# ericyao2013/path_planning_2d

Hardware: AMD Instinct MI355X
Metric: grid cells/sec for belief-update+Bellman loop, 1024x1024; plan step p50 ms (higher is better)
Workload: dtype fp32; 1 GPU; 1024x1024 cells per GPU: 1 belief update + 1 MDP Bellman sweep per step (BASELINE.json configs[2] grid); rows_per_gpu=1024, parallelism=single GPU, cells_per_lane=4, model=dictionary-coded (274 entries, uint16 code per cell)

## Files before the change

### path_planning_2d_amd/csrc/pp2_resident.hip

```cpp
#include <algorithm>
#include <cstring>
#include <type_traits>

#include "pp2_coded_dev.h"

namespace pp2 {

#ifdef PP2_RES_TRACE
__device__ unsigned long long g_rtrace[16][64][4][4];
#define PP2_RT(ph)                                                                    \
  if (tile < 16 && t < 64 && lane == 0 && (wave == 0 || wave == 5 || wave == 9 || wave == 12)) \
  g_rtrace[tile][t][wave == 0 ? 0 : wave == 5 ? 1 : wave == 9 ? 2 : 3][ph] =          \
      __builtin_amdgcn_s_memrealtime()
__device__ unsigned long long g_rtrace_pro[1024][8];
#define PP2_RP(ph) \
  if (tile < 1024 && threadIdx.x == 0) g_rtrace_pro[tile][ph] = __builtin_amdgcn_s_memrealtime()
#else
#define PP2_RT(ph) (void)0
#define PP2_RP(ph) (void)0
#endif

namespace {

typedef __amdgpu_buffer_rsrc_t Rsrc;
// ... 239 lines not shown
    if (sl < 0) continue;
#pragma unroll
    for (int k = 0; k < 4; ++k)
      p[k] = __builtin_fmaf(*reinterpret_cast<const float*>(qr + 4 * sl + cb[wr][k + 1 + wc]),
                            win.v[wr][k + 1 + wc], p[k]);
  }
#pragma unroll
  for (int k = 0; k < 4; ++k)
    p[k] = p[k] * *reinterpret_cast<const float*>(lt + __builtin_amdgcn_ubfe(lx4, 8 * k, 8));
}
__device__ __forceinline__ void belief_any_regs(int u, const ClassRegs& cr, uint32_t lx4, int z,
                                                const Win6& w, float (&p)[4]) {
  switch (u) {
#define PP2_BQ(UU)                               \
  case UU:                                       \
    belief_fact_regs<UU>(cr, lx4, z, w, p);      \
    break;
    PP2_BQ(0) PP2_BQ(1) PP2_BQ(2) PP2_BQ(3) PP2_BQ(4) PP2_BQ(5) PP2_BQ(6) PP2_BQ(7)
    default: belief_fact_regs<8>(cr, lx4, z, w, p);
#undef PP2_BQ
  }
}
__device__ __forceinline__ void load_class_regs(const uint8_t* sP, int prows, int ps, int ty,
                                                int x0, ClassRegs& cr) {
  const int lane = threadIdx.x & 63;
#pragma unroll
  for (int U = 0; U < 9; ++U)
#pragma unroll
    for (int oy = 0; oy < 3; ++oy) {
      const int sl = kCls.s[U][oy];
      if (sl < 0) continue;
      const uint8_t* r = sP + (U * prows + ty + oy) * ps + 4 + x0;
      const uint32_t m = *reinterpret_cast<const uint32_t*>(r);
      uint32_t e = 0u;
      if (lane == 0 || lane == 63) e = *reinterpret_cast<const uint32_t*>(r + (lane == 0 ? -4 : 4));
      const uint32_t l = (uint32_t)__builtin_amdgcn_update_dpp((int)e, (int)m, 0x138, 0xf, 0xf, false);
      const uint32_t h = (uint32_t)__builtin_amdgcn_update_dpp((int)e, (int)m, 0x130, 0xf, 0xf, false);
      cr.m[sl] = m;
      const uint32_t lh = (l >> 24) | ((h & 0xffu) << 8);
      cr.lh[sl / 2] = (sl & 1) ? cr.lh[sl / 2] | (lh << 16) : lh;
    }
}

template <bool TR>
__device__ __forceinline__ void belief_any(int u, const uint8_t* sP, int prows, int ps, int ty,
                                           int x0, uint32_t lx4, int z, const Win6& w,
                                           float (&p)[4]) {
  int off = (u * prows + ty) * ps;
  asm("" : "+v"(off));
  const uint8_t* pu = sP + off;
  switch (u) {
#define PP2_BQ(UU)                                                     \
  case UU:                                                             \
    belief_fact<UU, TR>(pu, ps, x0, lx4, z, w, p); \
    break;
    PP2_BQ(0) PP2_BQ(1) PP2_BQ(2) PP2_BQ(3) PP2_BQ(4) PP2_BQ(5) PP2_BQ(6) PP2_BQ(7)
    default: belief_fact<8, TR>(pu, ps, x0, lx4, z, w, p);
#undef PP2_BQ
  }
}
__device__ __forceinline__ const uint8_t* class_rows_of(int u, const uint8_t* sP, int prows, int ps,
                                                        int ty) {
  int off = (u * prows + ty) * ps;
  asm("" : "+v"(off));
  return sP + off;
}
template <bool TR>
__device__ __forceinline__ void belief_any_pre(int u, int x0, uint32_t lx4, int z, const Win6& w,
                                               const ClassRows& c, float (&p)[4]) {
  switch (u) {
#define PP2_BQ(UU)                                                  \
  case UU:                                                          \
    belief_fact<UU, TR, true>(nullptr, 0, x0, lx4, z, w, p, &c);    \
    break;
    PP2_BQ(0) PP2_BQ(1) PP2_BQ(2) PP2_BQ(3) PP2_BQ(4) PP2_BQ(5) PP2_BQ(6) PP2_BQ(7)
    default: belief_fact<8, TR, true>(nullptr, 0, x0, lx4, z, w, p, &c);
#undef PP2_BQ
  }
}

#ifndef PP2_RES_MASKED
#define PP2_RES_MASKED 1
#endif
template <int U>
__device__ __forceinline__ void belief_masked(float wm, float ws, const float (&tc)[4],
                                              const float (&lz)[4], const float (&mk)[4],
                                              const float (&bo)[4], const Win6& win,
                                              float (&p)[4]) {
#pragma unroll
  for (int k = 0; k < 4; ++k) p[k] = 0.0f;
#pragma unroll
  for (int s = 0; s < 9; ++s) {
    const int wr = s / 3, wc = s % 3 - 1, i = 8 - s;
    if (kSupSlot.s[U][i] < 0) continue;
#pragma unroll
    for (int k = 0; k < 4; ++k) {
      const float wt = i == 4 ? tc[k] : i == U ? wm : ws;
      p[k] = __builtin_fmaf(wt, win.v[wr][k + 1 + wc], p[k]);
    }
  }
#pragma unroll
  for (int k = 0; k < 4; ++k) {
    const float own = __builtin_fmaf(tc[k], bo[k], 0.0f);
    p[k] = (mk[k] == 0.0f ? own : p[k]) * lz[k];
  }
}
[[maybe_unused]] __device__ __forceinline__ void belief_any_masked(
    int u, float wm, float ws, const float (&tc)[4], const float (&lz)[4], const float (&mk)[4],
    const float (&bo)[4], const Win6& w, float (&p)[4]) {
  switch (u) {
#define PP2_BQ(UU)                                        \
  case UU:                                                \
    belief_masked<UU>(wm, ws, tc, lz, mk, bo, w, p);      \
    break;
    PP2_BQ(0) PP2_BQ(1) PP2_BQ(2) PP2_BQ(3) PP2_BQ(4) PP2_BQ(5) PP2_BQ(6) PP2_BQ(7)
    default: belief_masked<8>(wm, ws, tc, lz, mk, bo, w, p);
#undef PP2_BQ
  }
}
struct CentreSlots {
  unsigned long long v;
  constexpr CentreSlots() : v(0) {
    for (int u = 0; u < 9; ++u) v |= (unsigned long long)(4 * sup_slot(u, 4)) << (4 * u);
  }
};
constexpr CentreSlots kCentreSlot{};

__device__ __forceinline__ void row_lds(const float* row, int x0, float (&v)[6]) {
  const float* p = row + x0;
  const f4a m = *reinterpret_cast<const f4a*>(p);
  const int lane = threadIdx.x & 63;
  float e = 0.0f;
  if (lane == 0 || lane == 63) e = p[lane == 0 ? -1 : 4];
  v[0] = __int_as_float(__builtin_amdgcn_update_dpp(__float_as_int(e), __float_as_int(m[3]),
                                                    0x138, 0xf, 0xf, false));
  v[1] = m[0]; v[2] = m[1]; v[3] = m[2]; v[4] = m[3];
  v[5] = __int_as_float(__builtin_amdgcn_update_dpp(__float_as_int(e), __float_as_int(m[0]),
                                                    0x130, 0xf, 0xf, false));
}
__device__ __forceinline__ void row_zero(float (&v)[6]) {
#pragma unroll
  for (int i = 0; i < 6; ++i) v[i] = 0.0f;
}
#ifndef PP2_RES_WINDOW1
#define PP2_RES_WINDOW1 2
#endif
#ifndef PP2_RES_SWEEP_WINDOW1
#define PP2_RES_SWEEP_WINDOW1 PP2_RES_WINDOW1
#endif
#if PP2_RES_WINDOW1 != 0 || PP2_RES_SWEEP_WINDOW1 != 0
template <int NP>
struct WinRows {
  f4a q[NP][3];
  float e[NP][3];
};
template <int MODE, int NP>
__device__ __forceinline__ void issue_window_rows(const float* const (&p)[NP], int xs, bool in0,
                                                  bool in2, WinRows<NP>& w) {
  const int lane = threadIdx.x & 63;
#pragma unroll
  for (int k = 0; k < NP; ++k) w.q[k][1] = *reinterpret_cast<const f4a*>(p[k]);
  if (in0) {
#pragma unroll
    for (int k = 0; k < NP; ++k) w.q[k][0] = *reinterpret_cast<const f4a*>(p[k] - xs);
  }
  if (in2) {
#pragma unroll
    for (int k = 0; k < NP; ++k) w.q[k][2] = *reinterpret_cast<const f4a*>(p[k] + xs);
  }
  const int o0 = in0 ? -xs : 0, o2 = in2 ? xs : 0;
  auto edges = [&](int eo) {
#pragma unroll
    for (int k = 0; k < NP; ++k) w.e[k][2] = p[k][o2 + eo];
#pragma unroll
    for (int k = 0; k < NP; ++k) w.e[k][1] = p[k][eo];
#pragma unroll
    for (int k = NP - 1; k >= 0; --k) w.e[k][0] = p[k][o0 + eo];
  };
  if constexpr (MODE == 1) {
#pragma unroll
    for (int k = 0; k < NP; ++k)
#pragma unroll
      for (int r = 0; r < 3; ++r) w.e[k][r] = 0.0f;
    if (lane == 0 || lane == 63) edges(lane == 0 ? -1 : 4);
  } else {
    edges(lane < 32 ? -1 - 4 * lane : 4 + 4 * (63 - lane));
  }
}
__device__ __forceinline__ void window_row(const f4a& m, float e, float (&v)[6]) {
  v[0] = __int_as_float(__builtin_amdgcn_update_dpp(__float_as_int(e), __float_as_int(m[3]),
                                                    0x138, 0xf, 0xf, false));
  v[1] = m[0]; v[2] = m[1]; v[3] = m[2]; v[4] = m[3];
  v[5] = __int_as_float(__builtin_amdgcn_update_dpp(__float_as_int(e), __float_as_int(m[0]),
                                                    0x130, 0xf, 0xf, false));
}
#endif

__device__ __forceinline__ int xch_gran(int ntiles, int wpr, int slot, int tl, int side, int w,
                                        int k, int ln) {
  return (((((slot * ntiles + tl) * 2 + side) * wpr + w) * kResidentGranules + k) * 64 + ln) * 16;
}
#ifndef PP2_RES_XCD_PLAIN
#define PP2_RES_XCD_PLAIN 1
#endif
#ifndef PP2_RES_EARLY
#define PP2_RES_EARLY 2
#endif
#ifndef PP2_RES_REDW0
#define PP2_RES_REDW0 1
#endif
#ifndef PP2_RES_XCD_AUX
#define PP2_RES_XCD_AUX 0
#endif
__device__ __forceinline__ int tile_xcd(int t, int n) {
  const int q = n / 8, r = n % 8;
  return t < r * (q + 1) ? t / (q + 1) : r + (q > 0 ? (t - r * (q + 1)) / q : 0);
}
__device__ __forceinline__ void st_quad_x(Rsrc r, int off, const float (&v)[4], unsigned bit,
                                          bool plain) {
  const unsigned m = bit << 31;
  const u4v t = {__float_as_uint(v[0]) | m, __float_as_uint(v[1]) | m, __float_as_uint(v[2]) | m,
                 __float_as_uint(v[3]) | m};
  if (plain) __builtin_amdgcn_raw_buffer_store_b128(t, r, off, 0, PP2_RES_XCD_AUX);
  else __builtin_amdgcn_raw_buffer_store_b128(t, r, off, 0, kSc1);
}
__device__ __forceinline__ bool tagged(const u4v& g, unsigned m) {
  return (((g[0] ^ m) | (g[1] ^ m) | (g[2] ^ m) | (g[3] ^ m)) >> 31) == 0u;
}
__device__ __forceinline__ float untag(unsigned w) { return __uint_as_float(w & 0x7fffffffu); }
template <int NG>
__device__ __forceinline__ void take_granules(Rsrc r, int o, bool edge, int eo, unsigned bit,
                                              u4v (&g)[NG], unsigned (&e)[NG], unsigned* err,
                                              unsigned* err_host) {
  const unsigned m = bit << 31;
  const unsigned long long t0 = wall_clock64();
#pragma unroll
  for (int k = 0; k < NG; ++k) e[k] = m;
  for (int spin = 0;; ++spin) {
#pragma unroll
    for (int k = 0; k < NG; ++k) g[k] = __builtin_amdgcn_raw_buffer_load_b128(r, o + 1024 * k, 0, kSc1);
    if (edge) {
#pragma unroll
      for (int k = 0; k < NG; ++k) e[k] = __builtin_amdgcn_raw_buffer_load_b32(r, eo + 1024 * k, 0, kSc1);
    }
    bool ok = true;
#pragma unroll
    for (int k = 0; k < NG; ++k) ok = ok && tagged(g[k], m) && ((e[k] ^ m) >> 31) == 0u;
    if (__all(ok)) break;
    if ((spin & 7) == 7) {
      if (ld_flag(err) != 0u || wall_clock64() - t0 > kSpinTicks) {
        if ((threadIdx.x & 63) == 0) raise_err(err, err_host);
        return;
      }
    }
    __builtin_amdgcn_s_sleep(1);
    asm volatile("" ::: "memory");
  }
}
typedef unsigned u2v __attribute__((ext_vector_type(2)));
__device__ __forceinline__ int side_gran(int sbase, int ntiles, int slot, int tl, int side, int r) {
  return sbase + (((slot * ntiles + tl) * 2 + side) * kResidentMaxRt + r) * 8;
}
__device__ __forceinline__ void st_pair(Rsrc r, int off, float b, float j, unsigned bit) {
  const unsigned m = bit << 31;
  const u2v t = {__float_as_uint(b) | m, __float_as_uint(j) | m};
  __builtin_amdgcn_raw_buffer_store_b64(t, r, off, 0, kSc1);
}
__device__ __forceinline__ void take_rows_sides(Rsrc r, bool rows, int o, bool edge, int eo,
                                                bool sd, const int (&so)[3], int soff, unsigned bit,
                                                u4v (&g)[2], unsigned (&e)[2], u2v (&s)[3],
                                                unsigned* err, unsigned* err_host) {
  const unsigned m = bit << 31;
  const unsigned long long t0 = wall_clock64();
  e[0] = e[1] = m;
#pragma unroll
  for (int k = 0; k < 3; ++k) s[k] = u2v{m, m};
#ifdef PP2_RES_NOXCH
  g[0] = g[1] = u4v{m, m, m, m};
  return;
#endif
  for (int spin = 0;; ++spin) {
    if (rows) {
      g[0] = __builtin_amdgcn_raw_buffer_load_b128(r, o, 0, kSc1);
      g[1] = __builtin_amdgcn_raw_buffer_load_b128(r, o + 1024, 0, kSc1);
      if (edge) {
        e[0] = __builtin_amdgcn_raw_buffer_load_b32(r, eo, 0, kSc1);
        e[1] = __builtin_amdgcn_raw_buffer_load_b32(r, eo + 1024, 0, kSc1);
      }
    }
    if (sd) {
#pragma unroll
      for (int k = 0; k < 3; ++k)
        if (so[k] >= 0) s[k] = __builtin_amdgcn_raw_buffer_load_b64(r, so[k], soff, kSc1);
    }
    bool ok = true;
    if (rows)
      ok = tagged(g[0], m) && tagged(g[1], m) && (((e[0] ^ m) | (e[1] ^ m)) >> 31) == 0u;
#pragma unroll
    for (int k = 0; k < 3; ++k) ok = ok && (((s[k][0] ^ m) | (s[k][1] ^ m)) >> 31) == 0u;
#ifdef PP2_RES_NOWAIT
    ok = true;
#endif
    if (__all(ok)) break;
    if ((spin & 7) == 7) {
      if (ld_flag(err) != 0u || wall_clock64() - t0 > kSpinTicks) {
        if ((threadIdx.x & 63) == 0) raise_err(err, err_host);
        return;
      }
    }
    __builtin_amdgcn_s_sleep(1);
    asm volatile("" ::: "memory");
  }
}
__device__ __forceinline__ void row_quad(const float (&m)[4], float e, float (&v)[6]) {
  v[0] = __int_as_float(__builtin_amdgcn_update_dpp(__float_as_int(e), __float_as_int(m[3]),
                                                    0x138, 0xf, 0xf, false));
  v[1] = m[0]; v[2] = m[1]; v[3] = m[2]; v[4] = m[3];
  v[5] = __int_as_float(__builtin_amdgcn_update_dpp(__float_as_int(e), __float_as_int(m[0]),
                                                    0x130, 0xf, 0xf, false));
}

template <int CAP>
struct alignas(4) Trajectory {
  static_assert(CAP % 4 == 0, "the loop reads the trajectory as 32-bit words");
  uint8_t uz[CAP];
};

__device__ __forceinline__ ResidentMasked masked_arg() { return ResidentMasked{}; }
[[maybe_unused]] __device__ __forceinline__ ResidentMasked masked_arg(const ResidentMasked& m) {
  return m;
}
template <int CAP, int TC, bool LAG, bool TR, class... MW>
__global__ __launch_bounds__(TC == 3 ? 768 : 1024, TC == 3 ? 3 : 4) void k_loop_resident(
    const ResidentHead a, const Trajectory<CAP> tr, const MW... mwa) {
  static_assert(!TR || TC == 1, "transposed tiles are whole kernel rows");
  constexpr bool MSK = sizeof...(MW) != 0;
  static_assert(!MSK || (TC == 1 && !LAG && !TR), "the masked form is a whole-row instance");
  const ResidentMasked mw = masked_arg(mwa...);
  (void)mw;
  constexpr int kSweepG = TC == 3 ? 4 : TC > 1 ? 2 : 0;
  constexpr bool kSweepPipe = TC == 1 && !LAG && !TR;
  extern __shared__ __attribute__((aligned(16))) float lds[];
  constexpr int tc = TC == 3 ? 2 : TC;
  const int wp = a.g.wp, rows = a.g.rows, tw = wp / tc;
  const int tpr = tw >> 2, wpr = tw >> 8;
  const int xs = tw + 4;
  const int bufn = 4 + a.rt * xs;
  const int prows = a.rt + 2, ps = tw + 8;
  float* sTC = lds + lds_span(kResTab);
  uint8_t* sP = reinterpret_cast<uint8_t*>(sTC + lds_span(rows_floats(a.E, true)));
  float* sB0 = reinterpret_cast<float*>(sP) + lds_span(MSK ? kResGCn : 9 * prows * ps / 4);
  const float* sGC = reinterpret_cast<const float*>(sP);
  (void)sGC;
  float* sS = sB0 + 4 * bufn;
  float* sRed = sS + 16;

  const int tile = xcd_remap(blockIdx.x, gridDim.x);
  if (tile == a.stall_tile) return;
  const int trow = tile / tc, cx = tile - trow * tc, gx = cx * tw;
  PP2_RP(0);
  const unsigned prior_err = ld_flag(a.sync + kResidentSyncErr);
  const int lane = threadIdx.x & 63, wave = threadIdx.x >> 6;
  const int ty = __builtin_amdgcn_readfirstlane(threadIdx.x / tpr);
  const int wraw = __builtin_amdgcn_readfirstlane((threadIdx.x % tpr) >> 6);
  const int wj = tc > 1 ? __builtin_amdgcn_readfirstlane((wraw + ty) % wpr) : wraw;
  const int x0 = wj * 256 + lane * 4;
  const int y = trow * a.rt + ty;
  const bool valid = y < rows;
  const bool own = TR ? x0 >= a.own0 && x0 < a.own1 : y >= a.own0 && y < a.own1;
  auto hoff = [&](int yy, int xx) -> long long {
    return TR ? (long long)xx * a.ows + yy : (long long)yy * wp + xx;
  };
  const bool nb_up = valid && ty == 0 && trow > 0;
  const bool nb_dn = valid && ty == a.rt - 1 && y + 1 < rows;
  const bool sd_l = valid && wj == 0 && cx > 0;
  const bool sd_r = valid && wj == wpr - 1 && cx + 1 < tc;
  const bool sd_lane = (sd_l && lane == 0) || (sd_r && lane == 63);
  const int sbase = 2 * a.ntiles * 2 * (wp >> 8) * kResidentGranules * 64 * 16;
  unsigned* const err = a.sync + kResidentSyncErr;
  const Rsrc rx = make_rsrc(a.xch);
  auto sbuf = [&](int k, int slot) { return sB0 + (2 * k + slot) * bufn + 4; };
  const int myx = tile_xcd(tile, (int)gridDim.x);
  const bool plain_up = PP2_RES_XCD_PLAIN && nb_up && tile_xcd(tile - tc, (int)gridDim.x) == myx;
  const bool plain_dn = PP2_RES_XCD_PLAIN && nb_dn && tile_xcd(tile + tc, (int)gridDim.x) == myx;
  auto publish = [&](int slot, const float (&b)[4], const float (&j)[4], unsigned bit) {
#pragma unroll
    for (int side = 0; side < 2; ++side) {
      if (side == 0 ? !nb_up : !nb_dn) continue;
      const int o = xch_gran(a.ntiles, wpr, slot, tile, side, wj, 0, lane);
      const bool plain = side == 0 ? plain_up : plain_dn;
      st_quad_x(rx, o, b, bit, plain);
      st_quad_x(rx, o + 1024, j, bit, plain);
    }
    if (sd_lane) {
      const int o = side_gran(sbase, a.ntiles, slot, tile, sd_l ? 0 : 1, ty);
      if (sd_l) st_pair(rx, o, b[0], j[0], bit);
      else st_pair(rx, o, b[3], j[3], bit);
    }
  };
  int so[3] = {-1, -1, -1};
  if (tc > 1 && sd_lane) {
    const int dir = sd_l ? -1 : 1, nside = sd_l ? 1 : 0;
#pragma unroll
    for (int k = 0; k < 3; ++k) {
      const int rr = ty + k - 1, yy = y + k - 1;
      if (yy < 0 || yy >= rows) continue;
      const int tl2 = rr < 0 ? tile - tc + dir : rr >= a.rt ? tile + tc + dir : tile + dir;
      so[k] = side_gran(sbase, a.ntiles, 0, tl2, nside, rr < 0 ? a.rt - 1 : rr >= a.rt ? 0 : rr);
    }
  }
  const int sslot = a.ntiles * 2 * kResidentMaxRt * 8;
  auto take = [&](int slot, bool rows_in, int tl, int side, bool sd, unsigned bit, float (&vb)[6],
                  float (&vj)[6], float (&sb)[3], float (&sj)[3]) {
    const bool el = lane == 0 && wj > 0, er = lane == 63 && wj + 1 < wpr;
    const int o = xch_gran(a.ntiles, wpr, slot, tl, side, wj, 0, lane);
    const int eo = el ? xch_gran(a.ntiles, wpr, slot, tl, side, wj - 1, 0, 63) + 12
                      : xch_gran(a.ntiles, wpr, slot, tl, side, wj + 1, 0, 0);
    u4v g[2];
    unsigned e[2];
    u2v s[3];
    take_rows_sides(rx, rows_in, o, el || er, eo, sd && sd_lane, so, slot * sslot, bit, g, e, s,
                    err, a.err_host);
    if (rows_in) {
      const float mb[4] = {untag(g[0][0]), untag(g[0][1]), untag(g[0][2]), untag(g[0][3])};
      const float mj[4] = {untag(g[1][0]), untag(g[1][1]), untag(g[1][2]), untag(g[1][3])};
      row_quad(mb, (el || er) ? untag(e[0]) : 0.0f, vb);
      row_quad(mj, (el || er) ? untag(e[1]) : 0.0f, vj);
    }
    if (sd) {
#pragma unroll
      for (int k = 0; k < 3; ++k) {
        sb[k] = untag(s[k][0]);
        sj[k] = untag(s[k][1]);
      }
    }
  };

  const bool start0 = a.kstep0 % a.depth == 0;
  const bool red0 = start0 && a.in_partials && wave == 0;
  const bool red0_regs = red0 && a.in_n <= kPrologueParts;
  f4a pq[kPrologueParts / 256];
  if (red0_regs) {
    const f4a* q = reinterpret_cast<const f4a*>(a.in_partials);
    const int nq = a.in_n >> 2;
#pragma unroll
    for (int j = 0; j < kPrologueParts / 256; ++j) {
      const int i = lane + 64 * j;
      pq[j] = q[i < nq ? i : 0];
    }
  }
  f4a b_t = {0.0f, 0.0f, 0.0f, 0.0f}, j_t = {0.0f, 0.0f, 0.0f, 0.0f};
  if (valid) {
    if (TR) {
#pragma unroll
      for (int k = 0; k < 4; ++k) {
        b_t[k] = a.b_in[hoff(y, x0 + k)];
        j_t[k] = a.j_in[hoff(y, x0 + k)];
      }
    } else {
      const long long off = (long long)y * wp + gx + x0;
      b_t = *reinterpret_cast<const f4a*>(a.b_in + off);
      j_t = *reinterpret_cast<const f4a*>(a.j_in + off);
    }
  }
  stage_rows(a.rfact, kResTab, lds);
  stage_rows(a.rows, rows_floats(a.E, true), sTC);
  if constexpr (MSK) stage_rows(a.rfact + kResGC, kResGCn, reinterpret_cast<float*>(sP));
  for (int i = threadIdx.x; i < 4 * (a.rt + 1); i += blockDim.x) {
    const int buf = i / (a.rt + 1), r = i % (a.rt + 1);
    *reinterpret_cast<f4a*>(sB0 + buf * bufn + r * xs) = f4a{0.0f, 0.0f, 0.0f, 0.0f};
  }
  uint32_t cc[4] = {0u, 0u, 0u, 0u}, iwr[4][3], lx4 = 0u;
  if (valid) {
    if (TR) {
#pragma unroll
      for (int k = 0; k < 4; ++k) cc[k] = a.code[hoff(y, x0 + k)];
    } else {
      const uint2 m = *reinterpret_cast<const uint2*>(a.code + (long long)y * wp + gx + x0);
      cc[0] = m.x & 0xffffu; cc[1] = m.x >> 16; cc[2] = m.y & 0xffffu; cc[3] = m.y >> 16;
    }
    const uint8_t* lx = reinterpret_cast<const uint8_t*>(a.rfact + kResLX);
#pragma unroll
    for (int k = 0; k < 4; ++k) lx4 |= (uint32_t)lx[cc[k]] << (8 * k);
  }
  float mk[4] = {1.0f, 1.0f, 1.0f, 1.0f};
  if constexpr (MSK) {
    if (valid) {
      const uint8_t* fx = reinterpret_cast<const uint8_t*>(a.rfact + kResFX);
#pragma unroll
      for (int k = 0; k < 4; ++k) mk[k] = fx[cc[k]] ? 0.0f : 1.0f;
    }
  }
  __syncthreads();
  PP2_RP(1);
#pragma unroll
  for (int k = 0; k < 4; ++k) {
    const uint4 w = *reinterpret_cast<const uint4*>(sTC + kFactIW + 4 * cc[k]);
    iwr[k][0] = w.x; iwr[k][1] = w.y; iwr[k][2] = w.z;
  }
  for (int i = threadIdx.x; !MSK && i < prows * tpr; i += blockDim.x) {
    const int r = i / tpr, xq = (i % tpr) * 4, yy = trow * a.rt + r - 1;
    uint32_t pl[9] = {0u, 0u, 0u, 0u, 0u, 0u, 0u, 0u, 0u};
    if (yy >= 0 && yy < rows) {
      uint32_t c4[4];
      if (TR) {
#pragma unroll
        for (int k = 0; k < 4; ++k) c4[k] = a.code[hoff(yy, xq + k)];
      } else {
        const uint2 m = *reinterpret_cast<const uint2*>(a.code + (long long)yy * wp + gx + xq);
        c4[0] = m.x & 0xffffu; c4[1] = m.x >> 16; c4[2] = m.y & 0xffffu; c4[3] = m.y >> 16;
      }
#pragma unroll
      for (int k = 0; k < 4; ++k) {
        const uint4 w = *reinterpret_cast<const uint4*>(sTC + kFactIW + 4 * c4[k]);
#pragma unroll
        for (int q = 0; q < 9; ++q) {
          const uint32_t wq = q < 4 ? w.x : q < 8 ? w.y : w.z;
          pl[q] |= __builtin_amdgcn_ubfe(wq, 8 * (q % 4), 8) << (8 * k);
        }
      }
    }
#pragma unroll
    for (int q = 0; q < 9; ++q)
      *reinterpret_cast<uint32_t*>(sP + (q * prows + r) * ps + 4 + xq) = pl[q];
  }
  for (int i = threadIdx.x; !MSK && i < 9 * prows; i += blockDim.x) {
    const int q = i / prows, yy = trow * a.rt + i % prows - 1;
    uint32_t lp = 0u, rp = 0u;
    if (yy >= 0 && yy < rows) {
      auto cls = [&](int x) {
        const uint4 w = *reinterpret_cast<const uint4*>(
            sTC + kFactIW + 4 * a.code[hoff(yy, x)]);
        return __builtin_amdgcn_ubfe(q < 4 ? w.x : q < 8 ? w.y : w.z, 8 * (q % 4), 8);
      };
      if (gx > 0) lp = cls(gx - 1) << 24;
      if (gx + tw < wp) rp = cls(gx + tw);
    }
    *reinterpret_cast<uint32_t*>(sP + i * ps) = lp;
    *reinterpret_cast<uint32_t*>(sP + i * ps + 4 + tw) = rp;
  }
  PP2_RP(4);
  ClassRegs creg;
  if constexpr (TC == 3 && PP2_RES_HOIST) {
    __syncthreads();
    if (valid) load_class_regs(sP, prows, ps, ty, x0, creg);
  }
  if (prior_err != 0u) return;
  const bool bnd = nb_up || nb_dn || sd_l || sd_r;
  if (valid) {
    f4a b = b_t, j = j_t;
    if constexpr (MSK) {
      *reinterpret_cast<f4a*>(sbuf(0, 1) + ty * xs + x0) = b;
      *reinterpret_cast<f4a*>(sbuf(1, 1) + ty * xs + x0) = j;
#pragma unroll
      for (int k = 0; k < 4; ++k) {
        b[k] = b[k] * mk[k];
        j[k] = j[k] * mk[k];
      }
    }
    *reinterpret_cast<f4a*>(sbuf(0, 0) + ty * xs + x0) = b;
    *reinterpret_cast<f4a*>(sbuf(1, 0) + ty * xs + x0) = j;
    if (bnd) {
      const float bv[4] = {b[0], b[1], b[2], b[3]}, jv[4] = {j[0], j[1], j[2], j[3]};
      publish(1, bv, jv, (a.slot_use[1] + 1u) & 1u);
    }
  }
  unsigned use[2] = {a.slot_use[0], a.slot_use[1] + 1u};
  PP2_RP(5);
  if constexpr (kSweepPipe && PP2_RES_EARLY == 2) {
    if (threadIdx.x == 0) sS[1] = 0.0f;
  }
  if (red0) {
    float S;
    if (red0_regs) {
      const int nq = a.in_n >> 2;
      float sl = 0.0f;
#pragma unroll
      for (int j = 0; j < kPrologueParts / 256; ++j)
        if (lane + 64 * j < nq) sl += ((pq[j][0] + pq[j][1]) + pq[j][2]) + pq[j][3];
      S = wave_sum(sl);
    } else {
      S = wave_reduce_partials(a.in_partials, a.in_n);
    }
    if (threadIdx.x == 0) {
      sS[0] = S;
      if (tile == 0 && a.in_sum_out) *a.in_sum_out = S;
    }
  }
  __syncthreads();
  float inv = 1.0f;
  if (start0)
    inv = (1.0f / (a.in_partials ? sS[0] : a.in_sum ? *a.in_sum : 1.0f)) * a.bscale;

  const int pi = y * (wp >> 8) + cx * wpr + wj;
  const int redw = kSweepPipe && PP2_RES_REDW0 != 0 ? 0 : a.rt >= 3 && wpr >= 4 ? wpr + 1 : 0;
  unsigned arrivals = a.arrive_base;
  const unsigned nvw = kSweepPipe ? (unsigned)(std::min(a.rt, rows - trow * a.rt) * wpr) : 0u;
  unsigned early_n = 0u;
  (void)nvw;
  (void)early_n;
  int shift = 0;
  constexpr bool lag = LAG;
  int sh_prev = 0;
  unsigned arr_v = 0u;
  bool red_ok = false;
  auto lag_start = [&](int T) {
    return lag && T > 0 && T < a.n && T % a.depth == 0 && T - 1 - a.depth >= 0;
  };
  auto lag_target = [&](int T) { return a.arrive_base + (unsigned)(T / a.depth - 1) * a.ntiles; };
  float p[4] = {0.0f, 0.0f, 0.0f, 0.0f}, best[4] = {0.0f, 0.0f, 0.0f, 0.0f}, local = 0.0f;
  uint32_t arg[4] = {0u, 0u, 0u, 0u};
  if constexpr (MSK) {
    if (valid) {
      const f4a b = *reinterpret_cast<const f4a*>(sbuf(0, 1) + ty * xs + x0);
      const f4a j = *reinterpret_cast<const f4a*>(sbuf(1, 1) + ty * xs + x0);
#pragma unroll
      for (int k = 0; k < 4; ++k) {
        p[k] = b[k];
        best[k] = j[k];
      }
    }
  }
  PP2_RP(2);

  const uint32_t* const trw = reinterpret_cast<const uint32_t*>(tr.uz);
  uint32_t uzw = trw[0];
  int ph = a.kstep0 % a.depth;
  (void)trw;
  (void)uzw;
  (void)ph;
  for (int t = 0; t < a.n; ++t) {
#if PP2_RES_TRAJ_SGPR
    const uint32_t uzb = (uzw >> (8 * (t & 3))) & 0xffu;
    const int u = uzb & 15, z = uzb >> 4;
#else
    const int u = tr.uz[t] & 15, z = tr.uz[t] >> 4;
#endif
    const int ci = t & 1, co = ci ^ 1;
    const bool last = t == a.n - 1;
#if PP2_RES_PHASE_CTR
    const bool bs = t > 0 && ph == 0;
    ph = ph + 1 == a.depth ? 0 : ph + 1;
#else
    const bool bs = t > 0 && (a.kstep0 + t) % a.depth == 0;
#endif
    if (t > 0 && !bs) inv = 1.0f;
    if (lag) {
      if (wave == redw) {
        if (lag_start(t + 1)) {
          red_ok = a.red_lds && reached(arr_v, lag_target(t + 1));
          if (red_ok) {
            const float* src = a.ring + (size_t)((t - a.depth) % kResidentRing) * a.nparts;
            const int nq = a.nparts >> 2;
            for (int c = 0; c * 64 < nq; ++c) {
              const int i = c * 64 + lane < nq ? c * 64 + lane : nq - 1;
              __builtin_amdgcn_global_load_lds((glb_void*)(src + 4 * i), (lds_void*)(sRed + c * 256), 16,
                                               0, kSc1);
            }
          }
        }
        if (lag_start(t + 2)) arr_v = ld_flag(a.sync + kResidentSyncArrive);
      }
      if (bs) {
        const int sh = t - 1 - a.depth >= 0 ? pow2_shift_lagged(sS[0], sh_prev)
                       : start0 && (a.in_partials || a.in_sum) ? pow2_shift_lagged(a.bscale, 0)
                                                               : 0;
        sh_prev = sh;
        shift += sh;
        inv = pow2f(sh);
      }
    }
    PP2_RT(0);
    local = 0.0f;
#if PP2_RES_PHASE_CTR
    const bool arrive = ph == 0;
#else
    const bool arrive = (a.kstep0 + t + 1) % a.depth == 0;
#endif
    const bool mass = !kSweepPipe || arrive || last;
    const bool early = kSweepPipe && PP2_RES_EARLY != 0 && arrive && !bs && !last &&
                       !(t == 0 && start0);
    auto early_arrive = [&]() {
      float s = 0.0f;
#pragma unroll
      for (int k = 0; k < 4; ++k) s += p[k];
      const float v = wave_sum(s);
      if (lane == 0 && pi < a.nparts)
        st_flag(reinterpret_cast<unsigned*>(a.ring + (size_t)(t % kResidentRing) * a.nparts + pi),
                __float_as_uint(v));
      asm volatile("s_waitcnt vmcnt(0)" ::: "memory");
#if PP2_RES_EARLY == 1
      __syncthreads();
      if (threadIdx.x == 0)
        __hip_atomic_fetch_add(a.sync + kResidentSyncArrive, 1u, __ATOMIC_RELAXED,
                               __HIP_MEMORY_SCOPE_AGENT);
#else
      early_n += nvw;
      if (lane == 0) {
        const unsigned old = __hip_atomic_fetch_add(reinterpret_cast<unsigned*>(sS + 1), 1u,
                                                    __ATOMIC_RELAXED, __HIP_MEMORY_SCOPE_WORKGROUP);
        if (old + 1u == early_n)
          __hip_atomic_fetch_add(a.sync + kResidentSyncArrive, 1u, __ATOMIC_RELAXED,
                                 __HIP_MEMORY_SCOPE_AGENT);
      }
      asm volatile("" ::: "memory");
#endif
    };
    auto step_quad = [&]() {
      Win6 wb, wj;
      float sb[3] = {0.0f, 0.0f, 0.0f}, sj[3] = {0.0f, 0.0f, 0.0f};
      const bool sd = sd_l || sd_r;
      const unsigned bit = use[co] & 1u;
      ClassRows crow;
      if constexpr (kSweepPipe && !MSK)
        load_class_rows(class_rows_of(u, sP, prows, ps, ty), ps, x0, crow);
      float rtv[2][4][4], rcost[2][4];
      if constexpr (kSweepPipe && !MSK) {
        if (last) coded_sweep_iw_pipe_begin<4, true>(sTC, iwr, rtv, rcost, best, arg);
        else coded_sweep_iw_pipe_begin<4, false>(sTC, iwr, rtv, rcost, best, arg);
      }
      float tcv[4], lzv[4], mrec[2][4][2];
      if constexpr (MSK) {
        const char* qr = reinterpret_cast<const char*>(lds + kResQR) + u * (kFactK * 16) +
                         (int)((kCentreSlot.v >> (4 * u)) & 15u);
        const char* lt = reinterpret_cast<const char*>(lds + kResLT) + z * (kResLK * 4);
        const uint32_t sel0 = 0x0c0c0c00u | (uint32_t)(u & 7);
        const uint32_t sel1 = 0x0c0c0c00u | (u == 8 ? 4u : 0u);
#pragma unroll
        for (int k = 0; k < 4; ++k) {
          const uint32_t lo = __builtin_amdgcn_perm(iwr[k][1], iwr[k][0], sel0);
          tcv[k] = *reinterpret_cast<const float*>(qr + __builtin_amdgcn_perm(iwr[k][2], lo, sel1));
        }
#pragma unroll
        for (int k = 0; k < 4; ++k)
          lzv[k] = *reinterpret_cast<const float*>(lt + __builtin_amdgcn_ubfe(lx4, 8 * k, 8));
        if (last) masked_sweep_pipe_begin<4, true>(sGC, iwr, mrec);
        else masked_sweep_pipe_begin<4, false>(sGC, iwr, mrec);
      }
#if PP2_RES_WINDOW1 != 0
      if constexpr (kSweepPipe) {
        const bool in0 = ty > 0, in2 = ty + 1 < a.rt && y + 1 < rows;
        WinRows<2> wr;
        const float* const wp2[2] = {sbuf(0, ci) + ty * xs + x0, sbuf(1, ci) + ty * xs + x0};
        issue_window_rows<PP2_RES_WINDOW1>(wp2, xs, in0, in2, wr);
        __builtin_amdgcn_sched_barrier(0);
        if (in0) {
          window_row(wr.q[0][0], wr.e[0][0], wb.v[0]);
          window_row(wr.q[1][0], wr.e[1][0], wj.v[0]);
        } else if (nb_up) {
          take(co, true, tile - tc, 1, sd, bit, wb.v[0], wj.v[0], sb, sj);
        } else {
          row_zero(wb.v[0]);
          row_zero(wj.v[0]);
        }
        window_row(wr.q[0][1], wr.e[0][1], wb.v[1]);
        window_row(wr.q[1][1], wr.e[1][1], wj.v[1]);
        if (in2) {
          window_row(wr.q[0][2], wr.e[0][2], wb.v[2]);
          window_row(wr.q[1][2], wr.e[1][2], wj.v[2]);
        } else if (nb_dn) {
          take(co, true, tile + tc, 0, sd && !nb_up, bit, wb.v[2], wj.v[2], sb, sj);
        } else {
          row_zero(wb.v[2]);
          row_zero(wj.v[2]);
        }
      } else
#endif
      {
        if (ty > 0) {
          row_lds(sbuf(0, ci) + (ty - 1) * xs, x0, wb.v[0]);
          row_lds(sbuf(1, ci) + (ty - 1) * xs, x0, wj.v[0]);
        } else if (nb_up) {
          take(co, true, tile - tc, 1, sd, bit, wb.v[0], wj.v[0], sb, sj);
        } else {
          row_zero(wb.v[0]);
          row_zero(wj.v[0]);
        }
        row_lds(sbuf(0, ci) + ty * xs, x0, wb.v[1]);
        row_lds(sbuf(1, ci) + ty * xs, x0, wj.v[1]);
        if (ty + 1 < a.rt && y + 1 < rows) {
          row_lds(sbuf(0, ci) + (ty + 1) * xs, x0, wb.v[2]);
          row_lds(sbuf(1, ci) + (ty + 1) * xs, x0, wj.v[2]);
        } else if (nb_dn) {
          take(co, true, tile + tc, 0, sd && !nb_up, bit, wb.v[2], wj.v[2], sb, sj);
        } else {
          row_zero(wb.v[2]);
          row_zero(wj.v[2]);
        }
      }
      if (sd && !nb_up && !nb_dn) take(co, false, tile, 0, true, bit, wb.v[1], wj.v[1], sb, sj);
      if (sd_lane) {
#pragma unroll
        for (int k = 0; k < 3; ++k) {
          if (sd_l) {
            wb.v[k][0] = sb[k];
            wj.v[k][0] = sj[k];
          } else {
            wb.v[k][5] = sb[k];
            wj.v[k][5] = sj[k];
          }
        }
      }
      PP2_RT(1);
      if constexpr (TC == 3 && PP2_RES_HOIST) {
#pragma unroll
        for (int i = 0; i < kClsSlots; ++i) asm volatile("" : "+v"(creg.m[i]));
#pragma unroll
        for (int i = 0; i < (kClsSlots + 1) / 2; ++i) asm volatile("" : "+v"(creg.lh[i]));
        belief_any_regs(u, creg, lx4, z, wb, p);
      }
      else if constexpr (MSK) {
        const float bo[4] = {p[0], p[1], p[2], p[3]};
        belief_any_masked(u, mw.w_main, mw.w_side, tcv, lzv, mk, bo, wb, p);
        if constexpr (PP2_RES_EARLY != 0) {
          if (early) early_arrive();
        }
      }
      else if constexpr (kSweepPipe) {
        belief_any_pre<TR>(u, x0, lx4, z, wb, crow, p);
        if constexpr (PP2_RES_EARLY != 0) {
          if (early) early_arrive();
        }
      }
      else belief_any<TR>(u, sP, prows, ps, ty, x0, lx4, z, wb, p);
      float jn[9][4];
#pragma unroll
      for (int i = 0; i < 9; ++i)
#pragma unroll
        for (int k = 0; k < 4; ++k) jn[i][k] = TR ? wj.v[i % 3][k + i / 3] : wj.v[i / 3][k + i % 3];
      if constexpr (MSK) {
        float ov[4] = {best[0], best[1], best[2], best[3]};
        if (last)
          masked_sweep_pipe_rest<4, true>(sGC, iwr, jn, mw.gw_main, mw.gw_side, mrec, ov, best, arg);
        else
          masked_sweep_pipe_rest<4, false>(sGC, iwr, jn, mw.gw_main, mw.gw_side, mrec, ov, best, arg);
#pragma unroll
        for (int k = 0; k < 4; ++k) {
          const bool blocked = mk[k] == 0.0f;
          best[k] = blocked ? ov[k] : best[k];
          arg[k] = blocked ? 0u : arg[k];
        }
        *reinterpret_cast<f4a*>(sbuf(1, co) + ty * xs + x0) =
            f4a{best[0] * mk[0], best[1] * mk[1], best[2] * mk[2], best[3] * mk[3]};
        return;
      } else if constexpr (kSweepPipe) {
        if (last) coded_sweep_iw_pipe_rest<4, true>(sTC, iwr, jn, rtv, rcost, best, arg);
        else coded_sweep_iw_pipe_rest<4, false>(sTC, iwr, jn, rtv, rcost, best, arg);
      } else {
        if (last) coded_sweep_iw<4, true, kSweepG>(sTC, iwr, jn, best, arg);
        else coded_sweep_iw<4, false, kSweepG>(sTC, iwr, jn, best, arg);
      }
      *reinterpret_cast<f4a*>(sbuf(1, co) + ty * xs + x0) = f4a{best[0], best[1], best[2], best[3]};
    };
    auto finish_quad = [&]() {
#pragma unroll
      for (int k = 0; k < 4; ++k) p[k] = p[k] * inv;
      if (mass && !early) {
#pragma unroll
        for (int k = 0; k < 4; ++k) local += p[k];
      }
      if constexpr (MSK) {
        const float pm[4] = {p[0] * mk[0], p[1] * mk[1], p[2] * mk[2], p[3] * mk[3]};
        *reinterpret_cast<f4a*>(sbuf(0, co) + ty * xs + x0) = f4a{pm[0], pm[1], pm[2], pm[3]};
        if (bnd) {
          const float jm[4] = {best[0] * mk[0], best[1] * mk[1], best[2] * mk[2], best[3] * mk[3]};
          if (!last) publish(ci, pm, jm, (use[ci] + 1u) & 1u);
          __builtin_amdgcn_s_setprio(0);
        }
        return;
      }
      *reinterpret_cast<f4a*>(sbuf(0, co) + ty * xs + x0) = f4a{p[0], p[1], p[2], p[3]};
      if (bnd) {
        if (!last) publish(ci, p, best, (use[ci] + 1u) & 1u);
        __builtin_amdgcn_s_setprio(0);
      }
    };
    if (valid) {
      if (bnd) __builtin_amdgcn_s_setprio(2);
      step_quad();
      if (!bs || lag) finish_quad();
    }
#if PP2_RES_EARLY == 1
    else if (early) __syncthreads();
#endif
    if (bs && !lag) {
      if (wave == redw) {
        arrivals += a.ntiles;
        wave_wait(a.sync + kResidentSyncArrive, 1, arrivals, err, a.err_host);
        const float S = wave_reduce_partials_sc1(
            a.ring + (size_t)((t - 1) % kResidentRing) * a.nparts, a.nparts);
        if (lane == 0) sS[0] = S;
      }
      __syncthreads();
      if (a.shard) {
        const int sh = pow2_shift(sS[0]);
        shift += sh;
        inv = pow2f(sh);
      } else {
        inv = (1.0f / sS[0]) * a.bscale;
      }
      if (valid) finish_quad();
    }
    PP2_RT(2);
    if (last) break;
    ++use[ci];
    if (mass && !early) {
      const float v = wave_sum(local);
      if (lane == 0 && pi < a.nparts)
        st_flag(reinterpret_cast<unsigned*>(a.ring + (size_t)(t % kResidentRing) * a.nparts + pi),
                __float_as_uint(v));
    }
    if (arrive && !early) asm volatile("s_waitcnt vmcnt(0)" ::: "memory");
    if (wave == redw && lag_start(t + 1)) {
      float S;
      if (red_ok) {
        const int nq = a.nparts >> 2;
        float sl = 0.0f;
        for (int i = lane; i < nq; i += 64) {
          const f4a w = *reinterpret_cast<const f4a*>(sRed + 4 * i);
          sl += ((w[0] + w[1]) + w[2]) + w[3];
        }
        S = wave_sum(sl);
      } else {
        wave_wait(a.sync + kResidentSyncArrive, 1, lag_target(t + 1), err, a.err_host);
        S = wave_reduce_partials_sc1(a.ring + (size_t)((t - a.depth) % kResidentRing) * a.nparts,
                                     a.nparts);
      }
      if (lane == 0) sS[0] = S;
    }
#if PP2_RES_TRAJ_SGPR
    if (((t + 1) & 3) == 0 && t + 1 < CAP) uzw = trw[(t + 1) >> 2];
#endif
#ifndef PP2_RES_NOBAR
    __syncthreads();
#endif
    if (arrive && !early && threadIdx.x == 0)
      __hip_atomic_fetch_add(a.sync + kResidentSyncArrive, 1u, __ATOMIC_RELAXED,
                             __HIP_MEMORY_SCOPE_AGENT);
    PP2_RT(3);
  }

  if (own && TR) {
#pragma unroll
    for (int k = 0; k < 4; ++k) {
      const long long off = hoff(y, x0 + k);
      __builtin_nontemporal_store(p[k], a.b_out + off);
      __builtin_nontemporal_store(best[k], a.j_out + off);
      a.A[off] = (uint8_t)arg[k];
    }
  } else if (own) {
    const long long off = (long long)y * wp + gx + x0;
    store4<true>(a.b_out + off, p);
    store_ja<true>(a.j_out, a.A, off, best, arg);
  }
  const float v = wave_sum(own ? local : 0.0f);
  if (lane == 0 && pi < a.nparts) a.out_partials[pi] = v;
  if (a.scale_out && tile == 0 && threadIdx.x == 0) *a.scale_out = shift;
  PP2_RP(3);
}


__global__ __launch_bounds__(1024, 4) void k_sweep_resident(const SweepRun a) {
  extern __shared__ __attribute__((aligned(16))) float lds[];
  const int wp = a.g.wp, rows = a.g.rows, tpr = wp >> 2, wpr = wp >> 8;
  const int xs = wp + 4;
  const int bufn = 4 + a.rt * xs;
  float* sTC = lds;
  float* sJ0 = sTC + lds_span(rows_floats(a.E, true));
  float* sM = sJ0 + 3 * bufn;

  const int tile = xcd_remap(blockIdx.x, gridDim.x);
  if (tile == a.stall_tile) return;
  const unsigned prior_err = ld_flag(a.sync + kResidentSyncErr);
  const int lane = threadIdx.x & 63, wave = threadIdx.x >> 6;
  const int ty = __builtin_amdgcn_readfirstlane(threadIdx.x / tpr);
  const int wj = __builtin_amdgcn_readfirstlane((threadIdx.x % tpr) >> 6);
  const int x0 = (threadIdx.x % tpr) * 4;
// ... 106 lines not shown
      else if (nb_dn) take(co, tile + 1, 0, use[co] & 1u, w.v[2]);
      else row_zero(w.v[2]);
      float jn[9][4];
#pragma unroll
      for (int i = 0; i < 9; ++i)
#pragma unroll
        for (int k = 0; k < 4; ++k) jn[i][k] = w.v[i / 3][k + i % 3];
      if (check || fin) coded_sweep_iw_pipe<4, true>(sTC, iwr, jn, best, arg);
      else coded_sweep_iw_pipe<4, false>(sTC, iwr, jn, best, arg);
#endif
      *reinterpret_cast<f4a*>(sbuf(co) + ty * xs + x0) = f4a{best[0], best[1], best[2], best[3]};
      if (nb_up || nb_dn) {
        publish(ci, best, (use[ci] + 1u) & 1u);
        __builtin_amdgcn_s_setprio(0);
      }
    }
    ++use[ci];
    if (fin) break;
    if (!check) {
      __syncthreads();
      continue;
    }
    float m = 0.0f;
    if (valid) {
      float* sn = sbuf(2) + ty * xs + x0;
      const f4a old = *reinterpret_cast<const f4a*>(sn);
#pragma unroll
      for (int k = 0; k < 4; ++k) m = fmaxf(m, fabsf(old[k] - best[k]));
      *reinterpret_cast<f4a*>(sn) = f4a{best[0], best[1], best[2], best[3]};
    }
    m = wave_max(m);
    if (lane == 0) sM[wave] = m;
    __syncthreads();
    if (wave == 0) {
      float tm = lane < (int)(blockDim.x >> 6) ? sM[lane] : 0.0f;
      tm = wave_max(tm);
      if (lane == 0)
        st_flag(reinterpret_cast<unsigned*>(a.tile_max + (blk & 1) * a.ntiles + tile),
                __float_as_uint(tm));
      asm volatile("s_waitcnt vmcnt(0)" ::: "memory");
      if (lane == 0)
        __hip_atomic_fetch_add(a.sync + kResidentSyncArrive, 1u, __ATOMIC_RELAXED,
                               __HIP_MEMORY_SCOPE_AGENT);
      arrivals += a.ntiles;
      wave_wait(a.sync + kResidentSyncArrive, 1, arrivals, err, a.err_host);
      const Rsrc rm = make_rsrc(a.tile_max + (blk & 1) * a.ntiles);
      float g = 0.0f;
      for (int i = lane; i < a.ntiles; i += 64) g = fmaxf(g, ld1_sc1(rm, 4 * i));
      g = wave_max(g);
      if (lane == 0) sM[16] = g;
    }
    __syncthreads();
    norm = sM[16];
    ++blk;
    if (!((double)norm > a.thresh) || (a.cap_blocks > 0 && blk >= a.cap_blocks) ||
        blk >= a.max_blocks)
      break;
  }
  const int done = s + 1;
  if (valid) {
    store4<false>(a.j_out + goff, best);
    const uint32_t a4 = arg[0] | (arg[1] << 8) | (arg[2] << 16) | (arg[3] << 24);
    *reinterpret_cast<uint32_t*>(a.A + goff) = a4;
    if (a.nsweeps == 0)
      *reinterpret_cast<f4a*>(a.snap + goff) = f4a{best[0], best[1], best[2], best[3]};
  }
  if (tile == 0 && threadIdx.x == 0) {
    a.res[0] = done;
    a.res[1] = (int)__float_as_uint(norm);
  }
}

}

size_t resident_lds_bytes(const Geom& g, int E, int rt, int tc) {
  const int tw = g.wp / tc;
  return ((size_t)lds_span(kResTab) + lds_span(rows_floats(E, true)) +
          lds_span(9 * (rt + 2) * (tw + 8) / 4) + 4 * (4 + (size_t)rt * (tw + 4)) + 16) *
         sizeof(float);
}

size_t resident_masked_lds_bytes(const Geom& g, int E, int rt) {
  return ((size_t)lds_span(kResTab) + lds_span(rows_floats(E, true)) + lds_span(kResGCn) +
          4 * (4 + (size_t)rt * (g.wp + 4)) + 16) *
         sizeof(float);
}

bool resident_masked_built() { return PP2_RES_MASKED != 0; }

static int resident_tc(int tc, int threads) {
#ifndef PP2_RES_RICH
#define PP2_RES_RICH 1
#endif
  return tc == 2 && threads <= 768 && PP2_RES_RICH ? 3 : tc;
}

static bool resident_plan_tc(const Geom& g, int E, int ncus, int tc, ResidentPlan* p,
                             bool trn = false) {
  if (tc < 1 || tc > 2 || g.wp % (256 * tc) != 0 || (tc > 1 && g.wp / tc < 512) || ncus < tc) return false;
  const int rt = (g.rows + ncus / tc - 1) / (ncus / tc);
  const long long threads = (long long)rt * (g.wp / tc / 4);
  if (threads > 1024 || rt > kResidentMaxRt) return false;
  const size_t lds = resident_lds_bytes(g, E, rt, tc);
  if (lds > kDictLdsMaxBytes) return false;
  if (trn && tc != 1) return false;
  static unsigned long long attr[16] = {};
  const int ktc = resident_tc(tc, (int)threads);
#define PP2_K(CAPV, TCV, LAGV, TRV) reinterpret_cast<const void*>(&k_loop_resident<CAPV, TCV, LAGV, TRV>)
#define PP2_KT(CAPV, LAGV)                                                                    \
  (trn ? PP2_K(CAPV, 1, LAGV, true)                                                           \
       : ktc == 1 ? PP2_K(CAPV, 1, LAGV, false)                                               \
                  : ktc == 2 ? PP2_K(CAPV, 2, LAGV, false) : PP2_K(CAPV, 3, LAGV, false))
  const void* ks[4] = {PP2_KT(kResidentShortSteps, false), PP2_KT(kResidentMaxSteps, false),
                       PP2_KT(kResidentShortSteps, true), PP2_KT(kResidentMaxSteps, true)};
#undef PP2_KT
#undef PP2_K
  const int ai = trn ? 8 : 4 * (ktc - 1) + (ktc == 3 ? 4 : 0);
  int nb = 1 << 30;
  for (int k = 0; k < 4; ++k) {
    allow_lds(ks[k], attr[ai + k]);
    int n1 = 0;
    if (hipOccupancyMaxActiveBlocksPerMultiprocessor(&n1, ks[k], (int)threads, lds) != hipSuccess ||
        n1 < 1) {
      (void)hipGetLastError();
      return false;
    }
    nb = std::min(nb, n1);
  }
#if PP2_RES_MASKED
  if (ktc == 1 && !trn) {
    static unsigned long long mattr[2] = {};
    const void* km[2] = {
        reinterpret_cast<const void*>(
            &k_loop_resident<kResidentShortSteps, 1, false, false, ResidentMasked>),
        reinterpret_cast<const void*>(
            &k_loop_resident<kResidentMaxSteps, 1, false, false, ResidentMasked>)};
    for (int k = 0; k < 2; ++k) {
      allow_lds(km[k], mattr[k]);
      int n1 = 0;
      if (hipOccupancyMaxActiveBlocksPerMultiprocessor(&n1, km[k], (int)threads,
                                                       resident_masked_lds_bytes(g, E, rt)) !=
              hipSuccess ||
          n1 < 1) {
        (void)hipGetLastError();
        return false;
      }
      nb = std::min(nb, n1);
    }
  }
#endif
  p->rt = rt;
  p->tc = tc;
  p->tr = trn;
  p->ntiles = (g.rows + rt - 1) / rt * tc;
  p->threads = (int)threads;
  p->lds = lds;
  return (long long)nb * ncus >= p->ntiles;
}

bool resident_plan(const Geom& g, int E, int ncus, ResidentPlan* p, int tc_pref, bool allow_tr) {
  ResidentPlan p1, p2, pt;
  if (tc_pref == 3 && allow_tr && g.rows % 256 == 0 &&
      resident_plan_tc(transposed_geom(g), E, ncus, 1, &pt, true)) {
    *p = pt;
    return true;
  }
  const bool ok1 = resident_plan_tc(g, E, ncus, 1, &p1);
// ... 193 lines not shown
```

Measured before the change: 368.0 billion cells/s.

## Add lean padded LDS layout with branchless halo window loads for masked resident kernel

For the masked whole-row resident kernel, this pads the LDS tile buffers with zeroed guard rows and columns. The 3x3 window rows can then be read with unconditional loads, and neighbour halo rows are merged in by OR-ing exchange data over the loaded values, replacing the per-row boundary branches. It also keeps neighbour and plain-store role flags in a scalar register. It reuses the masked J product instead of recomputing it, and skips the arg clearing and shard-normalisation paths except where needed. The intent is to cut branch and divergence overhead and extra ALU work in the window and publish stages. The cost is a slightly larger LDS footprint, and the shard path is dropped in lean mode.

```diff
diff --git a/path_planning_2d_amd/csrc/pp2_resident.hip b/path_planning_2d_amd/csrc/pp2_resident.hip
--- a/path_planning_2d_amd/csrc/pp2_resident.hip
+++ b/path_planning_2d_amd/csrc/pp2_resident.hip
@@ -345,6 +345,13 @@
 #ifndef PP2_RES_MASKED
 #define PP2_RES_MASKED 1
 #endif
+#ifndef PP2_RES_LEAN
+#define PP2_RES_LEAN 1
+#endif
+#define PP2_RES_LEAN_ON (PP2_RES_LEAN != 0 && PP2_RES_WINDOW1 != 0)
+__host__ __device__ constexpr int lean_tile_floats(int rt, int tw) {
+  return 4 + (4 * (rt + 1) + 1) * (tw + 4);
+}
 template <int U>
 __device__ __forceinline__ void belief_masked(float wm, float ws, const float (&tc)[4],
                                               const float (&lz)[4], const float (&mk)[4],
@@ -449,6 +456,21 @@
   } else {
     edges(lane < 32 ? -1 - 4 * lane : 4 + 4 * (63 - lane));
   }
+}
+__device__ __forceinline__ void issue_window_rows_lean(const float* base, const int (&ro)[2][3],
+                                                       int xq, int xe, WinRows<2>& w) {
+#pragma unroll
+  for (int k = 0; k < 2; ++k) w.q[k][1] = *reinterpret_cast<const f4a*>(base + ro[k][1] + xq);
+#pragma unroll
+  for (int k = 0; k < 2; ++k) w.q[k][0] = *reinterpret_cast<const f4a*>(base + ro[k][0] + xq);
+#pragma unroll
+  for (int k = 0; k < 2; ++k) w.q[k][2] = *reinterpret_cast<const f4a*>(base + ro[k][2] + xq);
+#pragma unroll
+  for (int k = 0; k < 2; ++k) w.e[k][2] = base[ro[k][2] + xe];
+#pragma unroll
+  for (int k = 0; k < 2; ++k) w.e[k][1] = base[ro[k][1] + xe];
+#pragma unroll
+  for (int k = 1; k >= 0; --k) w.e[k][0] = base[ro[k][0] + xe];
 }
 __device__ __forceinline__ void window_row(const f4a& m, float e, float (&v)[6]) {
   v[0] = __int_as_float(__builtin_amdgcn_update_dpp(__float_as_int(e), __float_as_int(m[3]),
@@ -608,14 +630,15 @@
   const int wp = a.g.wp, rows = a.g.rows, tw = wp / tc;
   const int tpr = tw >> 2, wpr = tw >> 8;
   const int xs = tw + 4;
-  const int bufn = 4 + a.rt * xs;
+  constexpr bool kLean = MSK && PP2_RES_LEAN_ON;
+  const int bufn = kLean ? (a.rt + 1) * xs : 4 + a.rt * xs;
   const int prows = a.rt + 2, ps = tw + 8;
   float* sTC = lds + lds_span(kResTab);
   uint8_t* sP = reinterpret_cast<uint8_t*>(sTC + lds_span(rows_floats(a.E, true)));
   float* sB0 = reinterpret_cast<float*>(sP) + lds_span(MSK ? kResGCn : 9 * prows * ps / 4);
   const float* sGC = reinterpret_cast<const float*>(sP);
   (void)sGC;
-  float* sS = sB0 + 4 * bufn;
+  float* sS = sB0 + (kLean ? lean_tile_floats(a.rt, tw) : 4 * bufn);
   float* sRed = sS + 16;
 
   const int tile = xcd_remap(blockIdx.x, gridDim.x);
@@ -642,16 +665,25 @@
   const int sbase = 2 * a.ntiles * 2 * (wp >> 8) * kResidentGranules * 64 * 16;
   unsigned* const err = a.sync + kResidentSyncErr;
   const Rsrc rx = make_rsrc(a.xch);
-  auto sbuf = [&](int k, int slot) { return sB0 + (2 * k + slot) * bufn + 4; };
+  auto sbuf = [&](int k, int slot) { return sB0 + (2 * k + slot) * bufn + (kLean ? xs : 0) + 4; };
   const int myx = tile_xcd(tile, (int)gridDim.x);
   const bool plain_up = PP2_RES_XCD_PLAIN && nb_up && tile_xcd(tile - tc, (int)gridDim.x) == myx;
   const bool plain_dn = PP2_RES_XCD_PLAIN && nb_dn && tile_xcd(tile + tc, (int)gridDim.x) == myx;
+  enum : unsigned { kRoleUp = 1, kRoleDn = 2, kRolePlainUp = 4, kRolePlainDn = 8 };
+  unsigned role = 0u;
+  auto is = [&](unsigned bit, bool flag) {
+    if constexpr (kLean) {
+      asm volatile("" : "+s"(role));
+      return (role & bit) != 0u;
+    }
+    return flag;
+  };
   auto publish = [&](int slot, const float (&b)[4], const float (&j)[4], unsigned bit) {
 #pragma unroll
     for (int side = 0; side < 2; ++side) {
-      if (side == 0 ? !nb_up : !nb_dn) continue;
+      if (side == 0 ? !is(kRoleUp, nb_up) : !is(kRoleDn, nb_dn)) continue;
       const int o = xch_gran(a.ntiles, wpr, slot, tile, side, wj, 0, lane);
-      const bool plain = side == 0 ? plain_up : plain_dn;
+      const bool plain = side == 0 ? is(kRolePlainUp, plain_up) : is(kRolePlainDn, plain_dn);
       st_quad_x(rx, o, b, bit, plain);
       st_quad_x(rx, o + 1024, j, bit, plain);
     }
@@ -699,6 +731,29 @@
     }
   };
 
+  auto take_q = [&](int slot, int tl, int side, unsigned bit, f4a& qb, float& eb, f4a& qj,
+                    float& ej) {
+    const bool el = lane == 0 && wj > 0, er = lane == 63 && wj + 1 < wpr;
+    const int o = xch_gran(a.ntiles, wpr, slot, tl, side, wj, 0, lane);
+    const int eo = el ? xch_gran(a.ntiles, wpr, slot, tl, side, wj - 1, 0, 63) + 12
+                      : xch_gran(a.ntiles, wpr, slot, tl, side, wj + 1, 0, 0);
+    u4v g[2];
+    unsigned e[2];
+    u2v s[3];
+    take_rows_sides(rx, true, o, el || er, eo, false, so, 0, bit, g, e, s, err, a.err_host);
+    auto over = [](float z, unsigned w, unsigned keep) {
+      return __uint_as_float(__float_as_uint(z) | (w & keep));
+    };
+    const unsigned ke = (el || er) ? 0x7fffffffu : 0u;
+#pragma unroll
+    for (int k = 0; k < 4; ++k) {
+      qb[k] = over(qb[k], g[0][k], 0x7fffffffu);
+      qj[k] = over(qj[k], g[1][k], 0x7fffffffu);
+    }
+    eb = over(eb, e[0], ke);
+    ej = over(ej, e[1], ke);
+  };
+
   const bool start0 = a.kstep0 % a.depth == 0;
   const bool red0 = start0 && a.in_partials && wave == 0;
   const bool red0_regs = red0 && a.in_n <= kPrologueParts;
@@ -729,9 +784,13 @@
   stage_rows(a.rfact, kResTab, lds);
   stage_rows(a.rows, rows_floats(a.E, true), sTC);
   if constexpr (MSK) stage_rows(a.rfact + kResGC, kResGCn, reinterpret_cast<float*>(sP));
-  for (int i = threadIdx.x; i < 4 * (a.rt + 1); i += blockDim.x) {
+  for (int i = threadIdx.x; !kLean && i < 4 * (a.rt + 1); i += blockDim.x) {
     const int buf = i / (a.rt + 1), r = i % (a.rt + 1);
     *reinterpret_cast<f4a*>(sB0 + buf * bufn + r * xs) = f4a{0.0f, 0.0f, 0.0f, 0.0f};
+  }
+  if constexpr (kLean) {
+    for (int i = threadIdx.x; 4 * i < lean_tile_floats(a.rt, tw); i += blockDim.x)
+      *reinterpret_cast<f4a*>(sB0 + 4 * i) = f4a{0.0f, 0.0f, 0.0f, 0.0f};
   }
   uint32_t cc[4] = {0u, 0u, 0u, 0u}, iwr[4][3], lx4 = 0u;
   if (valid) {
@@ -810,6 +869,10 @@
   }
   if (prior_err != 0u) return;
   const bool bnd = nb_up || nb_dn || sd_l || sd_r;
+  if constexpr (kLean)
+    role = (unsigned)__builtin_amdgcn_readfirstlane(
+        (int)((nb_up ? kRoleUp : 0u) | (nb_dn ? kRoleDn : 0u) | (plain_up ? kRolePlainUp : 0u) |
+              (plain_dn ? kRolePlainDn : 0u)));
   if (valid) {
     f4a b = b_t, j = j_t;
     if constexpr (MSK) {
@@ -892,6 +955,8 @@
   (void)trw;
   (void)uzw;
   (void)ph;
+  const int xe = kLean ? wj * 256 + (lane < 32 ? -1 : 256) : 0;
+  (void)xe;
   for (int t = 0; t < a.n; ++t) {
 #if PP2_RES_TRAJ_SGPR
     const uint32_t uzb = (uzw >> (8 * (t & 3))) & 0xffu;
@@ -969,6 +1034,8 @@
       asm volatile("" ::: "memory");
 #endif
     };
+    float jmq[4] = {0.0f, 0.0f, 0.0f, 0.0f};
+    (void)jmq;
     auto step_quad = [&]() {
       Win6 wb, wj;
       float sb[3] = {0.0f, 0.0f, 0.0f}, sj[3] = {0.0f, 0.0f, 0.0f};
@@ -1001,7 +1068,25 @@
         else masked_sweep_pipe_begin<4, false>(sGC, iwr, mrec);
       }
 #if PP2_RES_WINDOW1 != 0
-      if constexpr (kSweepPipe) {
+      if constexpr (kLean) {
+        int ro[2][3];
+#pragma unroll
+        for (int k = 0; k < 2; ++k)
+#pragma unroll
+          for (int r = 0; r < 3; ++r) ro[k][r] = (2 * k + ci) * bufn + 4 + (ty + r) * xs;
+        WinRows<2> wr;
+        issue_window_rows_lean(sB0, ro, x0, xe, wr);
+        __builtin_amdgcn_sched_barrier(0);
+        if (nb_up)
+          take_q(co, tile - tc, 1, bit, wr.q[0][0], wr.e[0][0], wr.q[1][0], wr.e[1][0]);
+        if (nb_dn)
+          take_q(co, tile + tc, 0, bit, wr.q[0][2], wr.e[0][2], wr.q[1][2], wr.e[1][2]);
+#pragma unroll
+        for (int r = 0; r < 3; ++r) {
+          window_row(wr.q[0][r], wr.e[0][r], wb.v[r]);
+          window_row(wr.q[1][r], wr.e[1][r], wj.v[r]);
+        }
+      } else if constexpr (kSweepPipe) {
         const bool in0 = ty > 0, in2 = ty + 1 < a.rt && y + 1 < rows;
         WinRows<2> wr;
         const float* const wp2[2] = {sbuf(0, ci) + ty * xs + x0, sbuf(1, ci) + ty * xs + x0};
@@ -1101,7 +1186,13 @@
         for (int k = 0; k < 4; ++k) {
           const bool blocked = mk[k] == 0.0f;
           best[k] = blocked ? ov[k] : best[k];
-          arg[k] = blocked ? 0u : arg[k];
+          if (!kLean || last) arg[k] = blocked ? 0u : arg[k];
+        }
+        if constexpr (kLean) {
+#pragma unroll
+          for (int k = 0; k < 4; ++k) jmq[k] = best[k] * mk[k];
+          *reinterpret_cast<f4a*>(sbuf(1, co) + ty * xs + x0) = f4a{jmq[0], jmq[1], jmq[2], jmq[3]};
+          return;
         }
         *reinterpret_cast<f4a*>(sbuf(1, co) + ty * xs + x0) =
             f4a{best[0] * mk[0], best[1] * mk[1], best[2] * mk[2], best[3] * mk[3]};
@@ -1126,7 +1217,9 @@
         const float pm[4] = {p[0] * mk[0], p[1] * mk[1], p[2] * mk[2], p[3] * mk[3]};
         *reinterpret_cast<f4a*>(sbuf(0, co) + ty * xs + x0) = f4a{pm[0], pm[1], pm[2], pm[3]};
         if (bnd) {
-          const float jm[4] = {best[0] * mk[0], best[1] * mk[1], best[2] * mk[2], best[3] * mk[3]};
+          float jm[4];
+#pragma unroll
+          for (int k = 0; k < 4; ++k) jm[k] = kLean ? jmq[k] : best[k] * mk[k];
           if (!last) publish(ci, pm, jm, (use[ci] + 1u) & 1u);
           __builtin_amdgcn_s_setprio(0);
         }
@@ -1155,7 +1248,7 @@
         if (lane == 0) sS[0] = S;
       }
       __syncthreads();
-      if (a.shard) {
+      if (!kLean && a.shard) {
         const int sh = pow2_shift(sS[0]);
         shift += sh;
         inv = pow2f(sh);
@@ -1428,7 +1521,9 @@
 
 size_t resident_masked_lds_bytes(const Geom& g, int E, int rt) {
   return ((size_t)lds_span(kResTab) + lds_span(rows_floats(E, true)) + lds_span(kResGCn) +
-          4 * (4 + (size_t)rt * (g.wp + 4)) + 16) *
+          (PP2_RES_LEAN_ON ? (size_t)lean_tile_floats(rt, g.wp)
+                                                     : 4 * (4 + (size_t)rt * (g.wp + 4))) +
+          16) *
          sizeof(float);
 }
 
```

After: 385.5 billion cells/s, median of 6. 4.8% higher.
